# dphoyes/OpenCL-Structure-from-Motion

Hardware: AMD Instinct MI355X
Metric: stereo frame-pairs/sec (1242x375) through pushBack+matchFeatures(2), p_matched bit-exact (higher is better)
Workload: dtype u8

## Files before the change

### opencl-structure-from-motion_amd/csrc/vsm_feat.h

```cpp
#pragma once

#include <stdint.h>

#if defined(__HIPCC__)
#define VF_HD __host__ __device__ __forceinline__
#define VF_HDM __host__ __device__ __forceinline__
#else
#define VF_HD static inline __attribute__((always_inline))
#define VF_HDM inline __attribute__((always_inline))
#endif

typedef short vf_s2 __attribute__((ext_vector_type(2)));

VF_HD uint32_t vf_perm(uint32_t hi, uint32_t lo, uint32_t sel) {
#if defined(__HIP_DEVICE_COMPILE__)
  return __builtin_amdgcn_perm(hi, lo, sel);
#else
  const uint64_t src = ((uint64_t)hi << 32) | lo;
  uint32_t r = 0;
  for (int k = 0; k < 4; k++) {
    const uint32_t s = (sel >> (8 * k)) & 0xffu;
    const uint32_t b = s <= 7u ? (uint32_t)((src >> (8 * s)) & 0xffu) : 0u;
    r |= b << (8 * k);
  }
// ... 279 lines not shown
  const uint32_t t0 = vf_all(dy == 0), t1 = vf_all(dy == 1), t2 = vf_all(dy == 2);
  const uint32_t b3 = vf_all(dyb >= 3), b2 = vf_all(dyb == 2), b1 = vf_all(dyb == 1);
  uint32_t col[5];
#pragma unroll
  for (int c = 0; c < 5; c++) {
    const vf_s2 s2 = vf_pair(R[2][c]), s1 = vf_mm<MAX>(vf_pair(R[1][c]), s2), s0 = vf_mm<MAX>(vf_pair(R[0][c]), s1);
    const vf_s2 p7 = vf_pair(R[7][c]), p8 = vf_mm<MAX>(p7, vf_pair(R[8][c])), p9 = vf_mm<MAX>(p8, vf_pair(R[9][c]));
    const vf_s2 mid = vf_mm<MAX>(vf_mm<MAX>(vf_pair(R[3][c]), vf_pair(R[4][c])), vf_mm<MAX>(vf_pair(R[5][c]), vf_pair(R[6][c])));
    const uint32_t top = vf_bfi(t0, vf_bits(s0), vf_bfi(t1, vf_bits(s1), vf_bfi(t2, vf_bits(s2), neutral)));
    const uint32_t bot = vf_bfi(b3, vf_bits(p9), vf_bfi(b2, vf_bits(p8), vf_bfi(b1, vf_bits(p7), neutral)));
    col[c] = vf_bits(vf_mm<MAX>(vf_mm<MAX>(vf_pair(top), vf_pair(bot)), mid));
  }
  const uint32_t m0 = (vf_all(dx == 0) & 0x0000ffffu) | (vf_all(dx <= 1) & 0xffff0000u), m1 = vf_all(dx <= 2) | 0xffff0000u;
  const uint32_t m3 = vf_all(dxr >= 1) | 0x0000ffffu, m4 = (vf_all(dxr >= 2) & 0x0000ffffu) | (vf_all(dxr >= 3) & 0xffff0000u);
  vf_s2 w = vf_pair(col[2]);
  w = vf_mm<MAX>(w, vf_pair(vf_bfi(m0, col[0], neutral)));
  w = vf_mm<MAX>(w, vf_pair(vf_bfi(m1, col[1], neutral)));
  w = vf_mm<MAX>(w, vf_pair(vf_bfi(m3, col[3], neutral)));
  w = vf_mm<MAX>(w, vf_pair(vf_bfi(m4, col[4], neutral)));
  return MAX ? ((int)w.x > (int)w.y ? (int)w.x : (int)w.y) : ((int)w.x < (int)w.y ? (int)w.x : (int)w.y);
}

template <int STR>
VF_HD void vf_nms_dense_region(const int16_t *f, int li, int lj, int lim_i, int lim_j, int tau, int u0, int v0, int32_t &cmin,
                               int32_t &cmax) {
  static_assert((STR & 1) == 0, "plane rows must stay dword aligned");
  uint32_t R[10][5];
  {
    const uint32_t *base = (const uint32_t *)(f + (lj - 3) * STR + (li - 3));
#pragma unroll
    for (int r = 0; r < 10; r++) {
#pragma unroll
      for (int c = 0; c < 5; c++) R[r][c] = base[r * (STR / 2) + c];
    }
  }
  uint32_t kmin = 0xffffffffu, kmax = 0xffffffffu;
#pragma unroll
  for (int di = 0; di < 4; di++) {
#pragma unroll
    for (int dj = 0; dj < 4; dj++) {
      const int q = 3 + di;
      const uint32_t dw = R[3 + dj][q >> 1];
      const int val = (q & 1) ? ((int)dw >> 16) : (int)(short)(dw & 0xffffu);
      const uint32_t o = (uint32_t)(di * 4 + dj);
      const uint32_t a = ((uint32_t)(val + 32768) << 10) | o, b = ((uint32_t)(32767 - val) << 10) | o;
      kmin = a < kmin ? a : kmin;
      kmax = b < kmax ? b : kmax;
    }
  }
  const int mnv = (int)(kmin >> 10) - 32768, mno = (int)(kmin & 1023u);
  const int mxv = 32767 - (int)(kmax >> 10), mxo = (int)(kmax & 1023u);
  const int dxn = mno >> 2, dyn = mno & 3, dxx = mxo >> 2, dyx = mxo & 3;
  const int cx = lim_i - (li + 3), cy = lim_j - (lj + 3);
  const int wmn = vf_dense_window<false>(R, dxn, dyn, dxn < cx ? dxn : cx, dyn < cy ? dyn : cy);
  const int wmx = vf_dense_window<true>(R, dxx, dyx, dxx < cx ? dxx : cx, dyx < cy ? dyx : cy);
  const bool vmin = (mnv <= -tau) && wmn >= mnv, vmax = (mxv >= tau) && wmx <= mxv;
  cmin = vmin ? (int32_t)(0x80000000u | (uint32_t)(li + dxn + u0) | ((uint32_t)(lj + dyn + v0) << 14)) : 0;
  cmax = vmax ? (int32_t)(0x80000000u | (uint32_t)(li + dxx + u0) | ((uint32_t)(lj + dyx + v0) << 14)) : 0;
}

VF_HD void vf_dense_patch(const uint32_t *s_img, int16_t *s_f, int t, int tx, int ty, int bpl, int h, uint8_t *du_plane,
                          uint8_t *dv_plane, int16_t *dump_f1, int16_t *dump_f2) {
  typedef VfDense G;
  const int pr = t / G::PC, pc = t - pr * G::PC;
  VfWindow<G::ROWS> W;
  vf_load_window<G>(s_img, pc, pr, W);
  const int x0 = tx * G::TW + G::FX + 8 * pc, y0 = ty * G::TH + G::FY + G::ROWS * pr;
  const bool own = pc < G::PC_OWN && pr < G::PR_OWN && x0 >= 0 && x0 < bpl;
  int16_t *f1 = s_f + (G::ROWS * pr) * G::FS + 8 * pc, *f2 = f1 + G::FH * G::FS;
#pragma unroll
  for (int rr = 0; rr < G::ROWS; rr++) {
    const int y = y0 + rr;
    vf_s2 C3[6], C5[6], Cc[6], ctr[4], o1[4], o2[4];
#pragma unroll
    for (int j = 0; j < 6; j++) vf_columns_blob<G::ROWS>(W, rr, j, C3[j], C5[j], Cc[j]);
#pragma unroll
    for (int m = 0; m < 4; m++) ctr[m] = W.pair(rr + 2, m + 1);
    vf_blob_row(C3, C5, Cc, ctr, o1, o2);
    vf_store16(f1 + rr * G::FS, vf_bits(o1[0]), vf_bits(o1[1]), vf_bits(o1[2]), vf_bits(o1[3]));
    vf_store16(f2 + rr * G::FS, vf_bits(o2[0]), vf_bits(o2[1]), vf_bits(o2[2]), vf_bits(o2[3]));
    if (own && y >= 0 && y < h) {
      uint32_t du[2], dv[2];
      vf_s2 S[6], D[6];
#pragma unroll
      for (int j = 0; j < 6; j++) vf_columns_sobel<G::ROWS>(W, rr, j, S[j], D[j]);
      if (y < 3 || y > h - 4) vf_sobel_zero_outside(S, D, y * bpl + x0, 2 * bpl, (h - 2) * bpl);
      vf_sobel_row(S, D, du, dv);
      uint32_t *pu = (uint32_t *)(du_plane + (size_t)y * bpl + x0), *pv = (uint32_t *)(dv_plane + (size_t)y * bpl + x0);
      pu[0] = du[0], pu[1] = du[1];
      pv[0] = dv[0], pv[1] = dv[1];
      if (dump_f1) {
#pragma unroll
        for (int m = 0; m < 4; m++) {
          const int x = x0 + 2 * m;
          dump_f1[(size_t)y * bpl + x] = vf_f1_mask(x, y, bpl, h) ? o1[m].x : (short)0;
          dump_f1[(size_t)y * bpl + x + 1] = vf_f1_mask(x + 1, y, bpl, h) ? o1[m].y : (short)0;
          dump_f2[(size_t)y * bpl + x] = vf_f2_mask(x, y, bpl, h) ? o2[m].x : (short)0;
          dump_f2[(size_t)y * bpl + x + 1] = vf_f2_mask(x + 1, y, bpl, h) ? o2[m].y : (short)0;
        }
      }
    }
  }
}

VF_HD void vf_dense_nms(const int16_t *s_f, int it, int tx, int ty, int mw, int mh, int margin, int tau, int ncu, int ncv,
                        int32_t *cand) {
  typedef VfDense G;
  static_assert(G::CU == 32, "a cell row per half wave");
  const int lcu = it & 31, k = (it >> 5) & 1, lcv = it >> 6;
  const int ci = G::CU * tx + G::CELL_U0 + lcu, cj = G::CV * ty + G::CELL_V0 + lcv;
  const int u0 = tx * G::TW + G::FX, v0 = ty * G::TH + G::FY;
  const int lim_i = mw - 1 - margin - u0, lim_j = mh - 1 - margin - v0;
  int32_t cmin, cmax;
  vf_nms_dense_region<G::FS>(s_f + k * G::FH * G::FS, G::CELL_X0 + (G::N + 1) * lcu, G::CELL_Y0 + (G::N + 1) * lcv, lim_i, lim_j, tau, u0,
                             v0, cmin, cmax);
  if (ci >= 0 && ci < ncu && cj >= 0 && cj < ncv) {
    int32_t *c = cand + (size_t)(ci * ncv + cj) * 4 + 2 * k;
    c[0] = cmin;
    c[1] = cmax;
  }
}

struct VfSparseKeep {
  uint32_t f2[VfSparse::ROWS][4];
};
VF_HD void vf_sparse_patch(const uint32_t *s_img, int16_t *s_f, int t, VfSparseKeep &keep) {
  typedef VfSparse G;
  const int pr = t / G::PC, pc = t - pr * G::PC;
  VfWindow<G::ROWS> W;
  vf_load_window<G>(s_img, pc, pr, W);
  int16_t *f1 = s_f + (G::ROWS * pr) * G::FS + 8 * pc;
#pragma unroll
  for (int rr = 0; rr < G::ROWS; rr++) {
    vf_s2 C3[6], C5[6], Cc[6], ctr[4], o1[4], o2[4];
#pragma unroll
    for (int j = 0; j < 6; j++) vf_columns_blob<G::ROWS>(W, rr, j, C3[j], C5[j], Cc[j]);
#pragma unroll
    for (int m = 0; m < 4; m++) ctr[m] = W.pair(rr + 2, m + 1);
    vf_blob_row(C3, C5, Cc, ctr, o1, o2);
    vf_store16(f1 + rr * G::FS, vf_bits(o1[0]), vf_bits(o1[1]), vf_bits(o1[2]), vf_bits(o1[3]));
#pragma unroll
    for (int m = 0; m < 4; m++) keep.f2[rr][m] = vf_bits(o2[m]);
  }
}
VF_HD void vf_sparse_store_f2(int16_t *s_f, int t, const VfSparseKeep &keep) {
  typedef VfSparse G;
  const int pr = t / G::PC, pc = t - pr * G::PC;
  int16_t *f = s_f + (G::ROWS * pr) * G::FS + 8 * pc;
#pragma unroll
  for (int rr = 0; rr < G::ROWS; rr++) {
    vf_store16(f + rr * G::FS, keep.f2[rr][0], keep.f2[rr][1], keep.f2[rr][2], keep.f2[rr][3]);
  }
}
template <int LANES>
VF_HD void vf_sparse_nms(const int16_t *s_f, int it, int l8, int k, int tx, int ty, int mw, int mh, int margin, int tau, int ncu,
                         int ncv, int32_t *cand) {
  typedef VfSparse G;
  const int lcv = it / G::CU, lcu = it - lcv * G::CU;
  const int ci = G::CU * tx + G::CELL_U0 + lcu, cj = G::CV * ty + G::CELL_V0 + lcv;
  const int u0 = tx * G::TW + G::FX, v0 = ty * G::TH + G::FY;
  const int lim_i = mw - 1 - margin - u0, lim_j = mh - 1 - margin - v0;
  const bool fast = lim_i >= G::FW - 1 && lim_j >= G::FH - 1;
  int32_t cmin, cmax;
  const int li = G::CELL_X0 + (G::N + 1) * lcu, lj = G::CELL_Y0 + (G::N + 1) * lcv;
  if (fast)
    vf_nms_item<G::N, LANES, G::FS, true>(s_f, li, lj, l8, lim_i, lim_j, tau, u0, v0, cmin, cmax);
  else
    vf_nms_item<G::N, LANES, G::FS, false>(s_f, li, lj, l8, lim_i, lim_j, tau, u0, v0, cmin, cmax);
  if (l8 == 0 && ci < ncu && cj < ncv) {
    int32_t *c = cand + (size_t)(ci * ncv + cj) * 4 + 2 * k;
    c[0] = cmin;
    c[1] = cmax;
  }
}
```

### opencl-structure-from-motion_amd/csrc/vsm_image.hip

```cpp

#include <stdlib.h>

#include <algorithm>

#include "vsm_internal.h"
#include "vsm_dev.h"
#include "vsm_feat.h"

#ifdef VSM_FEAT_TIMING
__device__ unsigned int vsm_ft_rec[5][1 << 16][10];
extern "C" int vsm_debug_feat_rec(unsigned int *out, int reset) {
  if (hipMemcpyFromSymbol(out, HIP_SYMBOL(vsm_ft_rec), sizeof(vsm_ft_rec)) != hipSuccess) return -1;
  (void)reset;
  return 0;
}
#define FT_DECL unsigned long long ft_t[10]; int ft_n = 0
#define FT_STAMP ft_t[ft_n++] = __builtin_amdgcn_s_memtime()
#define FT_FLUSH(kern)                                                              \
  do {                                                                              \
    const unsigned wv = ((blockIdx.z * gridDim.y + blockIdx.y) * gridDim.x + blockIdx.x) * (blockDim.x >> 6) + (threadIdx.x >> 6); \
    if ((threadIdx.x & 63) == 0 && wv < (1u << 16)) {                               \
      vsm_ft_rec[kern][wv][0] = (unsigned)ft_t[0] | 1u;                             \
      for (int q = 1; q < ft_n; q++) vsm_ft_rec[kern][wv][q] = (unsigned)(ft_t[q] - ft_t[q - 1]); \
    }                                                                               \
// ... 489 lines not shown
}

template <int N, int TCU, int TCV, int LANES>
__global__ void __launch_bounds__(256)
    k_nms_fixed(const VsmImage *__restrict__ imgs, int first, VsmDims d, const int16_t *__restrict__ f1base,
                const int16_t *__restrict__ f2base, size_t f_stride, int tau, int si, int nbx, int n_img) {
  constexpr int N1 = N + 1, W = 2 * N + 1;
  constexpr int TW = TCU * N1 + 2 * N, TH = TCV * N1 + 2 * N;
  constexpr int STR = (((TW + 1) / 2) | 1) * 2;
  static_assert(TCU * TCV * 2 * LANES == 256, "one item per LANES threads");
  static_assert((N1 & 1) == 0, "tile origins must stay dword aligned");
  __shared__ int16_t s_f[2][TH][STR];
  const int lb = xcd_remap(blockIdx.x, gridDim.x);
  const int zi = lb / nbx, bx = lb - zi * nbx;
  if (zi >= n_img) return;
  const VsmSet &st = imgs[first + zi].set[si];
  const int tiles_u = (st.ncu + TCU - 1) / TCU;
  const int tu = bx % tiles_u, tv = bx / tiles_u;
  const int cu0 = tu * TCU, cv0 = tv * TCV;
  const int u0 = VSM_MARGIN + cu0 * N1, v0 = VSM_MARGIN + cv0 * N1;
  const int16_t *__restrict__ f1 = f1base + (size_t)zi * f_stride;
  const int16_t *__restrict__ f2 = f2base + (size_t)zi * f_stride;
  for (int e = threadIdx.x; e < (TW / 2) * TH; e += 256) {
    const int y = e / (TW / 2), x = 2 * (e - y * (TW / 2));
    const int u = u0 + x, v = v0 + y;
    const bool in = u + 1 < d.mbpl && v < d.mh;
    const uint32_t a = in ? *(const uint32_t *)(f1 + v * d.mbpl + u) : 0u;
    const uint32_t b = in ? *(const uint32_t *)(f2 + v * d.mbpl + u) : 0u;
    *(uint32_t *)&s_f[0][y][x] = a;
    *(uint32_t *)&s_f[1][y][x] = b;
  }
  __syncthreads();
  const int l8 = threadIdx.x % LANES, item = threadIdx.x / LANES;
  const int k = item & 1, cl = item >> 1;
  const int lcu = cl % TCU, lcv = cl / TCU;
  const int ci = cu0 + lcu, cj = cv0 + lcv;
  const bool live = ci < st.ncu && cj < st.ncv;
  const int16_t(*f)[STR] = s_f[k];
  const int li = N + lcu * N1, lj = N + lcv * N1;
  uint32_t kmin = 0xffffffffu, kmax = 0xffffffffu;
  {
    const int16_t *c0 = &f[lj][li];
#pragma unroll
    for (int t = 0; t < (N1 + LANES - 1) / LANES; t++) {
      const int di = l8 + t * LANES;
      if (di < N1) {
#pragma unroll
        for (int dj = 0; dj < N1; dj++) {
          const int val = c0[dj * STR + di];
          const uint32_t o = (uint32_t)(di * N1 + dj);
          kmin = min(kmin, ((uint32_t)(val + 32768) << 10) | o);
          kmax = min(kmax, ((uint32_t)(32767 - val) << 10) | o);
        }
      }
    }
  }
#pragma unroll
  for (int o = LANES / 2; o >= 1; o >>= 1) {
    kmin = min(kmin, (uint32_t)__shfl_xor((int)kmin, o, LANES));
    kmax = min(kmax, (uint32_t)__shfl_xor((int)kmax, o, LANES));
  }
  const int mnv = (int)(kmin >> 10) - 32768, mno = kmin & 1023;
  const int mxv = 32767 - (int)(kmax >> 10), mxo = kmax & 1023;
  const int mni = li + mno / N1, mnj = lj + mno % N1, mxi = li + mxo / N1, mxj = lj + mxo % N1;
  const int lim_i = d.mw - 1 - VSM_MARGIN - u0, lim_j = d.mh - 1 - VSM_MARGIN - v0;
  int wmn = 32767, wmx = -32768;
  if (lim_i >= TW - 1 && lim_j >= TH - 1) {
    typedef short vsm_s2 __attribute__((ext_vector_type(2)));
    constexpr int ND = (W + 1) / 2;
    const int cn = mni - N, cx = mxi - N;
    const bool pn1 = (cn & 1) != 0, px1 = (cx & 1) != 0;
    const uint32_t *pn = (const uint32_t *)&f[mnj - N][cn & ~1], *px = (const uint32_t *)&f[mxj - N][cx & ~1];
    vsm_s2 amn = {32767, 32767}, amx = {-32768, -32768};
#pragma unroll
    for (int t = 0; t < (W + LANES - 1) / LANES; t++) {
      const int r = l8 + t * LANES;
      if (r < W) {
        const uint32_t *rn = pn + r * (STR / 2), *rx = px + r * (STR / 2);
#pragma unroll
        for (int c = 0; c < ND; c++) {
          uint32_t vn = rn[c], vx = rx[c];
          if (c == 0) {
            vn = pn1 ? ((vn & 0xffff0000u) | 0x00007fffu) : vn;
            vx = px1 ? ((vx & 0xffff0000u) | 0x00008000u) : vx;
          }
          if (c == ND - 1) {
            vn = pn1 ? vn : ((vn & 0x0000ffffu) | 0x7fff0000u);
            vx = px1 ? vx : ((vx & 0x0000ffffu) | 0x80000000u);
          }
          amn = __builtin_elementwise_min(amn, __builtin_bit_cast(vsm_s2, vn));
          amx = __builtin_elementwise_max(amx, __builtin_bit_cast(vsm_s2, vx));
        }
      }
    }
    wmn = min((int)amn.x, (int)amn.y);
    wmx = max((int)amx.x, (int)amx.y);
  } else {
    for (int r = l8; r < W; r += LANES) {
      if (mnj - N + r <= lim_j)
        for (int c = 0; c < W && mni - N + c <= lim_i; c++) wmn = min(wmn, (int)f[mnj - N + r][mni - N + c]);
      if (mxj - N + r <= lim_j)
        for (int c = 0; c < W && mxi - N + c <= lim_i; c++) wmx = max(wmx, (int)f[mxj - N + r][mxi - N + c]);
    }
  }
#pragma unroll
  for (int o = LANES / 2; o >= 1; o >>= 1) {
    wmn = min(wmn, __shfl_xor(wmn, o, LANES));
    wmx = max(wmx, __shfl_xor(wmx, o, LANES));
  }
  if (live && l8 == 0) {
    const bool vmin = (mnv <= -tau) && wmn >= mnv, vmax = (mxv >= tau) && wmx <= mxv;
    int32_t *c = st.cand + (size_t)(ci * st.ncv + cj) * 4 + 2 * k;
    c[0] = vmin ? (int32_t)(0x80000000u | (uint32_t)(mni + u0) | ((uint32_t)(mnj + v0) << 14)) : 0;
    c[1] = vmax ? (int32_t)(0x80000000u | (uint32_t)(mxi + u0) | ((uint32_t)(mxj + v0) << 14)) : 0;
  }
}



template <bool DUMP>
__global__ void __launch_bounds__(256)
    k_feat_dense(const VsmImage *__restrict__ imgs, int first, VsmDims d, int tau, int tiles_x, int nbx, int n_img,
                 int16_t *__restrict__ f1base, int16_t *__restrict__ f2base, size_t f_stride) {
  typedef VfDense G;
  __shared__ __attribute__((aligned(16))) uint32_t s_img[G::IH * G::IWD];
  __shared__ __attribute__((aligned(16))) int16_t s_f[2 * G::FH * G::FS];
  const int lb = xcd_remap(blockIdx.x, gridDim.x);
  const int zi = lb / nbx, bx = lb - zi * nbx;
  if (zi >= n_img) return;
  const VsmImage &im = imgs[first + zi];
  const VsmSet &st = im.set[1];
  const int ty = bx / tiles_x, tx = bx - ty * tiles_x;
  const int t = threadIdx.x;
  FT_DECL;
  FT_STAMP;
  vf_fill<G, 256>(s_img, im.imgm, d.mbpl * d.mh, d.mbpl, tx, ty, t);
  FT_STAMP;
  __syncthreads();
  FT_STAMP;
  if (t < G::PC * G::PR)
    vf_dense_patch(s_img, s_f, t, tx, ty, d.mbpl, d.mh, im.du, im.dv, DUMP ? f1base + (size_t)zi * f_stride : nullptr,
                   DUMP ? f2base + (size_t)zi * f_stride : nullptr);
  FT_STAMP;
  __syncthreads();
  FT_STAMP;
  for (int it = t; it < G::CU * G::CV * 2; it += 256) vf_dense_nms(s_f, it, tx, ty, d.mw, d.mh, VSM_MARGIN, tau, st.ncu, st.ncv, st.cand);
  FT_STAMP;
  FT_FLUSH(0);
}

__global__ void __launch_bounds__(256)
    k_feat_sparse(const VsmImage *__restrict__ imgs, int first, VsmDims d, int tau, int tiles_x, int nbx, int n_img) {
  typedef VfSparse G;
  __shared__ __attribute__((aligned(16))) uint32_t s_img[G::IH * G::IWD];
  __shared__ __attribute__((aligned(16))) int16_t s_f[G::FH * G::FS];
  const int lb = xcd_remap(blockIdx.x, gridDim.x);
  const int zi = lb / nbx, bx = lb - zi * nbx;
  if (zi >= n_img) return;
  const VsmImage &im = imgs[first + zi];
  const VsmSet &st = im.set[0];
  const int ty = bx / tiles_x, tx = bx - ty * tiles_x;
  const int t = threadIdx.x;
  FT_DECL;
  FT_STAMP;
  vf_fill<G, 256>(s_img, im.imgm, d.mbpl * d.mh, d.mbpl, tx, ty, t);
  FT_STAMP;
  __syncthreads();
  FT_STAMP;
  VfSparseKeep keep;
  if (t < G::PC * G::PR) vf_sparse_patch(s_img, s_f, t, keep);
  FT_STAMP;
  __syncthreads();
  FT_STAMP;
  static_assert((G::CU * G::CV) % 32 == 0, "whole rounds of 32 items x 8 lanes");
  for (int it = t >> 3; it < G::CU * G::CV; it += 32) vf_sparse_nms<8>(s_f, it, t & 7, 0, tx, ty, d.mw, d.mh, VSM_MARGIN, tau, st.ncu, st.ncv, st.cand);
  FT_STAMP;
  __syncthreads();
  if (t < G::PC * G::PR) vf_sparse_store_f2(s_f, t, keep);
  __syncthreads();
  FT_STAMP;
  for (int it = t >> 3; it < G::CU * G::CV; it += 32) vf_sparse_nms<8>(s_f, it, t & 7, 1, tx, ty, d.mw, d.mh, VSM_MARGIN, tau, st.ncu, st.ncv, st.cand);
  FT_STAMP;
  FT_FLUSH(1);
}

static void vsm_feat_tiles(const VsmDims &d, const VsmSet &dense, int &dx, int &dy) {
  dx = std::max((d.mbpl + 8 + 127) / 128, (dense.ncu + 3 + 31) / 32);
  dy = std::max((d.mh + 4 + 47) / 48, (dense.ncv + 2 + 11) / 12);
}

__global__ void __launch_bounds__(1024) k_scan_cells(const VsmImage *__restrict__ imgs, int first, int set_lo, int nb) {
  __shared__ int s_w[17];
  const VsmSet &st = imgs[first + blockIdx.z].set[blockIdx.y];
  if ((int)blockIdx.y < set_lo) {
    if (threadIdx.x == 0) {
      *st.count = 0;
      *st.count_host = 0;
    }
    return;
  }
  for (int b = threadIdx.x; b < nb; b += 1024) st.bin_cnt[b] = 0;
  const int ncells = st.ncu * st.ncv;
  const int chunk = (ncells + 1023) / 1024;
  const int c0 = min((int)threadIdx.x * chunk, ncells), c1 = min(c0 + chunk, ncells);
  int sum = 0, total, run;
  if (chunk <= 8) {
    int cnt[8];
#pragma unroll
    for (int k = 0; k < 8; k++) {
      cnt[k] = 0;
      if (c0 + k < c1) {
        const int4 v = ldg_i4(st.cand + (size_t)(c0 + k) * 4);
        cnt[k] = (v.x < 0) + (v.y < 0) + (v.z < 0) + (v.w < 0);
      }
    }
#pragma unroll
    for (int k = 0; k < 8; k++) sum += cnt[k];
    run = block_excl_scan_1024(sum, total, s_w);
#pragma unroll
    for (int k = 0; k < 8; k++)
      if (c0 + k < c1) {
        st.cell_off[c0 + k] = run;
        run += cnt[k];
      }
  } else {
    for (int c = c0; c < c1; c++) {
      const int4 v = *(const int4 *)(st.cand + (size_t)c * 4);
      sum += (v.x < 0) + (v.y < 0) + (v.z < 0) + (v.w < 0);
    }
    run = block_excl_scan_1024(sum, total, s_w);
    for (int c = c0; c < c1; c++) {
      const int4 v = *(const int4 *)(st.cand + (size_t)c * 4);
      st.cell_off[c] = run;
      run += (v.x < 0) + (v.y < 0) + (v.z < 0) + (v.w < 0);
    }
  }
  if (threadIdx.x == 0) {
    st.cell_off[ncells] = total;
    *st.count = total;
    *st.count_host = total;
  }
}

__constant__ int8_t c_desc_dv[16] = {-1, +1, -1, +1, -1, +1, -1, +1, -5, +5, -5, +5, -3, +3, -3, +3};
__constant__ int8_t c_desc_du[16] = {-3, -3, -1, -1, +3, +3, +1, +1, -1, -1, +1, +1, -5, -5, +5, +5};

#define EMIT_TW 128
#define EMIT_TH 32
#define EMIT_HALO 5
#define EMIT_LW (EMIT_TW + 2 * EMIT_HALO + 4)
#define EMIT_LH (EMIT_TH + 2 * EMIT_HALO)
__global__ void __launch_bounds__(256) k_emit(const VsmImage *__restrict__ imgs, int first, VsmDims d, int set_lo,
                                              int binsize, int nbx, int n_img) {
  __shared__ uint16_t s_g[EMIT_LH][EMIT_LW + 2];
  const int lb = xcd_remap(blockIdx.x, gridDim.x);
  const int zi = lb / nbx, bx = lb - zi * nbx;
  if (zi >= n_img) return;
  const VsmImage &im = imgs[first + zi];
  const int si = blockIdx.y;
  if (si < set_lo) return;
  const VsmSet &st = im.set[si];
  const int n1 = st.nms_n + 1;
  const int tcu = max(EMIT_TW / n1, 1), tcv = max(EMIT_TH / n1, 1);
  const int tiles_u = (st.ncu + tcu - 1) / tcu, tiles_v = (st.ncv + tcv - 1) / tcv;
  if (bx >= tiles_u * tiles_v) return;
  const int tu = bx % tiles_u, tv = bx / tiles_u;
  const int cu0 = tu * tcu, cv0 = tv * tcv;
  const int ut = st.nms_n + VSM_MARGIN + cu0 * n1 - EMIT_HALO, vt = st.nms_n + VSM_MARGIN + cv0 * n1 - EMIT_HALO;
  const int ua = ut & ~3;
  const bool staged = n1 <= EMIT_TH;
  if (staged) {
    for (int e = threadIdx.x; e < (EMIT_LW / 4 + 1) * EMIT_LH; e += 256) {
      const int y = e / (EMIT_LW / 4 + 1), x = 4 * (e - y * (EMIT_LW / 4 + 1));
      const int u = ua + x, v = vt + y;
      if (x + 3 < EMIT_LW + 2) {
        uint32_t a = 0, b = 0;
        if (u >= 0 && u + 3 < d.mbpl && v >= 0 && v < d.mh) {
          a = ldg_u32(im.du + (size_t)v * d.mbpl + u);
          b = ldg_u32(im.dv + (size_t)v * d.mbpl + u);
        }
        const uint32_t lo = (a & 0xffu) | ((b & 0xffu) << 8) | ((a & 0xff00u) << 8) | ((b & 0xff00u) << 16);
        const uint32_t hi = ((a >> 16) & 0xffu) | (((b >> 16) & 0xffu) << 8) | ((a >> 24) << 16) | ((b >> 24) << 24);
        *(uint2 *)&s_g[y][x] = make_uint2(lo, hi);
      }
    }
    __syncthreads();
  }
  for (int t = threadIdx.x; t < tcu * tcv; t += 256) {
    const int lcv = t % tcv, lcu = t / tcv;
    const int ci = cu0 + lcu, cj = cv0 + lcv;
    if (ci >= st.ncu || cj >= st.ncv) continue;
    const int cell = ci * st.ncv + cj;
    const int4 c4 = ldg_i4(st.cand + (size_t)cell * 4);
    if ((c4.x | c4.y | c4.z | c4.w) >= 0) continue;
    const int cc4[4] = {c4.x, c4.y, c4.z, c4.w};
    int pos = ldg_i32(st.cell_off + cell);
#pragma unroll
    for (int g = 0; g < 4; g++) {
      const int cc = cc4[g];
      if (cc >= 0) continue;
      const int u = cc & 0x3fff, v = (cc >> 14) & 0x3fff;
      uint32_t t16[16];
      if (staged) {
        const uint16_t *c0 = &s_g[v - vt][u - ua];
#pragma unroll
        for (int m = 0; m < 16; m++) {
          constexpr int8_t kdv[16] = {-1, +1, -1, +1, -1, +1, -1, +1, -5, +5, -5, +5, -3, +3, -3, +3};
          constexpr int8_t kdu[16] = {-3, -3, -1, -1, +3, +3, +1, +1, -1, -1, +1, +1, -5, -5, +5, +5};
          t16[m] = c0[kdv[m] * (EMIT_LW + 2) + kdu[m]];
        }
      } else {
#pragma unroll
        for (int m = 0; m < 16; m++) {
          const int a = (v + c_desc_dv[m]) * d.mbpl + u + c_desc_du[m];
          t16[m] = (uint32_t)im.du[a] | ((uint32_t)im.dv[a] << 8);
        }
      }
      vsm_u4 r0, r1, r2;
      r0.x = (uint32_t)(u * d.scale);
      r0.y = (uint32_t)(v * d.scale);
      r0.z = 0u;
      r0.w = (uint32_t)g;
      r1.x = t16[0] | (t16[1] << 16);
      r1.y = t16[2] | (t16[3] << 16);
      r1.z = t16[4] | (t16[5] << 16);
      r1.w = t16[6] | (t16[7] << 16);
      r2.x = t16[8] | (t16[9] << 16);
      r2.y = t16[10] | (t16[11] << 16);
      r2.z = t16[12] | (t16[13] << 16);
      r2.w = t16[14] | (t16[15] << 16);
      VSM_AS1 vsm_u4 *rec = (VSM_AS1 vsm_u4 *)(st.feat + (size_t)pos * 12);
      rec[0] = r0;
      rec[1] = r1;
      rec[2] = r2;
// ... 534 lines not shown
```

Measured before the change: 55100.

## Replace per-cell sparse NMS with hierarchical block-level min/max pruning in shared memory

For interior tiles, the sparse-NMS stage now runs as several cooperative phases. Column min/max reductions feed per-block argmin records, and each cell decides from its 8 neighbour blocks whether it survives. Only ambiguous neighbour regions are queued as jobs for a row scan, and a fallback to the per-item path covers job-buffer overflow. The level structures reuse the image tile's LDS through a union to keep occupancy, at the cost of extra barriers, an atomic job counter and more complex control flow.

```diff
diff --git a/opencl-structure-from-motion_amd/csrc/vsm_feat.h b/opencl-structure-from-motion_amd/csrc/vsm_feat.h
--- a/opencl-structure-from-motion_amd/csrc/vsm_feat.h
+++ b/opencl-structure-from-motion_amd/csrc/vsm_feat.h
@@ -455,24 +455,225 @@
     vf_store16(f + rr * G::FS, keep.f2[rr][0], keep.f2[rr][1], keep.f2[rr][2], keep.f2[rr][3]);
   }
 }
-template <int LANES>
-VF_HD void vf_sparse_nms(const int16_t *s_f, int it, int l8, int k, int tx, int ty, int mw, int mh, int margin, int tau, int ncu,
-                         int ncv, int32_t *cand) {
+VF_HD bool vf_sparse_fast(int tx, int ty, int mw, int mh, int margin) {
+  typedef VfSparse G;
+  return mw - 1 - margin - (tx * G::TW + G::FX) >= G::FW - 1 && mh - 1 - margin - (ty * G::TH + G::FY) >= G::FH - 1;
+}
+template <int LANES, bool fast>
+VF_HD void vf_sparse_item(const int16_t *s_f, int it, int l8, int k, int tx, int ty, int mw, int mh, int margin, int tau, int ncu,
+                          int ncv, int32_t *cand) {
   typedef VfSparse G;
   const int lcv = it / G::CU, lcu = it - lcv * G::CU;
   const int ci = G::CU * tx + G::CELL_U0 + lcu, cj = G::CV * ty + G::CELL_V0 + lcv;
   const int u0 = tx * G::TW + G::FX, v0 = ty * G::TH + G::FY;
   const int lim_i = mw - 1 - margin - u0, lim_j = mh - 1 - margin - v0;
-  const bool fast = lim_i >= G::FW - 1 && lim_j >= G::FH - 1;
   int32_t cmin, cmax;
   const int li = G::CELL_X0 + (G::N + 1) * lcu, lj = G::CELL_Y0 + (G::N + 1) * lcv;
-  if (fast)
-    vf_nms_item<G::N, LANES, G::FS, true>(s_f, li, lj, l8, lim_i, lim_j, tau, u0, v0, cmin, cmax);
-  else
-    vf_nms_item<G::N, LANES, G::FS, false>(s_f, li, lj, l8, lim_i, lim_j, tau, u0, v0, cmin, cmax);
+  vf_nms_item<G::N, LANES, G::FS, fast>(s_f, li, lj, l8, lim_i, lim_j, tau, u0, v0, cmin, cmax);
   if (l8 == 0 && ci < ncu && cj < ncv) {
     int32_t *c = cand + (size_t)(ci * ncv + cj) * 4 + 2 * k;
     c[0] = cmin;
     c[1] = cmax;
   }
 }
+
+typedef uint32_t vf_u2a __attribute__((ext_vector_type(2), may_alias));
+struct alignas(16) VfLevels {
+  typedef VfSparse G;
+  static constexpr int N1 = G::N + 1, BU = G::CU + 2, BV = G::CV + 2, NB = BU * BV, ITEMS = G::CU * G::CV;
+  static constexpr int JOBS = 256;
+  static_assert(G::CELL_X0 - N1 >= 0 && G::CELL_X0 + N1 * (G::CU + 1) <= G::FW, "the ring's columns inside the plane");
+  static_assert(G::CELL_Y0 - G::N == 0 && G::CELL_Y0 + N1 * (G::CV + 1) <= G::FH, "the top ring from row 0, the bottom ring inside the plane");
+  static_assert(G::FS % 4 == 0 && G::FW < 256 && G::FH < 64 && 2 * ITEMS <= 128 && N1 <= 16, "columns in fours; the fields of a block's and a job's word");
+  int16_t col[2][BV][G::FS];
+  uint32_t blk[2][NB];
+  uint32_t jobs[JOBS + 1][2];
+  uint32_t keep[2 * ITEMS];
+  uint32_t full[ITEMS];
+  uint32_t njobs;
+  static VF_HDM int bx0(int bu) { return G::CELL_X0 + N1 * (bu - 1); }
+  static VF_HDM int by0(int bv) { return bv ? G::CELL_Y0 + N1 * (bv - 1) : 0; }
+  static VF_HDM int val16(uint32_t rec, int s) { return (int)(int16_t)(rec & 0xffffu) ^ s; }
+  static VF_HDM int px(uint32_t rec) { return (int)((rec >> 16) & 0xffu); }
+  static VF_HDM int py(uint32_t rec) { return (int)(rec >> 24); }
+};
+VF_HD uint32_t vf_levels_count(uint32_t *p, uint32_t n) {
+#if defined(__HIP_DEVICE_COMPILE__)
+  return atomicAdd(p, n);
+#else
+  const uint32_t v = *p;
+  *p = v + n;
+  return v;
+#endif
+}
+
+template <int NT>
+VF_HD void vf_levels_columns(const int16_t *f, VfLevels &L, int t) {
+  typedef VfLevels V;
+  constexpr int FS = VfSparse::FS, QW = FS / 4;
+  for (int e = t; e < V::BV * QW; e += NT) {
+    const int bv = e / QW, c = e - bv * QW;
+    const int16_t *p = f + V::by0(bv) * FS + 4 * c;
+    vf_u2a r = *(const vf_u2a *)p;
+    vf_s2 mn0 = vf_pair(r.x), mn1 = vf_pair(r.y), mx0 = mn0, mx1 = mn1;
+#pragma unroll
+    for (int i = 1; i < V::N1; i++) {
+      r = *(const vf_u2a *)(p + i * FS);
+      mn0 = __builtin_elementwise_min(mn0, vf_pair(r.x)), mn1 = __builtin_elementwise_min(mn1, vf_pair(r.y));
+      mx0 = __builtin_elementwise_max(mx0, vf_pair(r.x)), mx1 = __builtin_elementwise_max(mx1, vf_pair(r.y));
+    }
+    const vf_u2a mn = {vf_bits(mn0), vf_bits(mn1)}, mx = {vf_bits(mx0), vf_bits(mx1)};
+    *(vf_u2a *)(L.col[0][bv] + 4 * c) = mn;
+    *(vf_u2a *)(L.col[1][bv] + 4 * c) = mx;
+  }
+}
+
+VF_HD void vf_levels_blocks(const int16_t *f, VfLevels &L, int t) {
+  typedef VfLevels V;
+  if (t < V::ITEMS) L.full[t] = 0;
+  if (t == 0) L.njobs = 0;
+  if (t >= 2 * V::NB) return;
+  const int b = t >> 1, k = t & 1, s = -k;
+  const int bv = b / V::BU, bu = b - bv * V::BU;
+  const int x0 = V::bx0(bu), y0 = V::by0(bv);
+  const int16_t *col = L.col[k][bv] + x0;
+  int kx = 0x7fffffff, ky = 0x7fffffff;
+#pragma unroll
+  for (int i = 0; i < V::N1; i++) {
+    const int key = ((int)col[i] ^ s) * 16 + i;
+    kx = key < kx ? key : kx;
+  }
+  const int16_t *line = f + y0 * VfSparse::FS + x0 + (kx & 15);
+#pragma unroll
+  for (int i = 0; i < V::N1; i++) {
+    const int key = ((int)line[i * VfSparse::FS] ^ s) * 16 + i;
+    ky = key < ky ? key : ky;
+  }
+  L.blk[k][b] = ((uint32_t)((ky >> 4) ^ s) & 0xffffu) | ((uint32_t)(x0 + (kx & 15)) << 16) | ((uint32_t)(y0 + (ky & 15)) << 24);
+}
+
+VF_HD void vf_levels_decide(VfLevels &L, int t, int tau) {
+  typedef VfLevels V;
+  if (t >= 2 * V::ITEMS) return;
+  const int it = t >> 1, k = t & 1, s = -k;
+  const int lcv = it / VfSparse::CU, lcu = it - lcv * VfSparse::CU;
+  const uint32_t *blk = L.blk[k] + lcv * V::BU + lcu;
+  const uint32_t own = blk[V::BU + 1];
+  const int v = V::val16(own, s), cx = V::px(own), cy = V::py(own);
+  const int li = V::bx0(lcu + 1), lj = V::by0(lcv + 1), N = VfSparse::N;
+  const int wl = li - cx + N, wr = cx - li, hu = lj - cy + N, hd = cy - lj;
+  const uint32_t xpart[3] = {(uint32_t)(cx - N) | (uint32_t)(wl - 1) << 14, (uint32_t)li | 9u << 14, (uint32_t)(li + V::N1) | (uint32_t)(wr - 1) << 14};
+  const uint32_t ypart[3] = {(uint32_t)(cy - N) << 8 | (uint32_t)(hu - 1) << 18, (uint32_t)lj << 8 | 9u << 18,
+                             (uint32_t)(lj + V::N1) << 8 | (uint32_t)(hd - 1) << 18};
+  const bool some_x[3] = {wl > 0, true, wr > 0}, some_y[3] = {hu > 0, true, hd > 0};
+  bool open = v <= (k ? ~tau : -tau);
+  uint32_t need = 0;
+#pragma unroll
+  for (int n = 0; n < 8; n++) {
+    const int q = n + (n >= 4), du = q % 3, dv = q / 3;
+    const uint32_t r = blk[dv * V::BU + du];
+    const int nx = V::px(r), ny = V::py(r);
+    const bool better = V::val16(r, s) < v;
+    const bool inside = (du == 0 ? nx >= cx - N : du == 2 ? nx <= cx + N : true) && (dv == 0 ? ny >= cy - N : dv == 2 ? ny <= cy + N : true);
+    open = open && !(better && inside);
+    need |= (uint32_t)(better && !inside && some_x[du] && some_y[dv]) << n;
+  }
+  L.keep[t] = open;
+  if (!open || !need) return;
+  const uint32_t base = vf_levels_count(&L.njobs, (uint32_t)__builtin_popcount(need));
+  uint32_t j = base;
+#pragma unroll
+  for (int n = 0; n < 8; n++) {
+    if ((need >> n) & 1u) {
+      const int q = n + (n >= 4);
+      const vf_u2a job = {xpart[q % 3] | ypart[q / 3] | (uint32_t)t << 22, (uint32_t)v};
+      *(vf_u2a *)L.jobs[j < (uint32_t)V::JOBS ? j : (uint32_t)V::JOBS] = job;
+      j++;
+    }
+  }
+  if (j > (uint32_t)V::JOBS) L.full[it] = 1;
+}
+
+template <int NT, int JL>
+VF_HD void vf_levels_scan(const int16_t *f, VfLevels &L, int t) {
+  typedef VfLevels V;
+  const uint32_t nj = L.njobs < (uint32_t)V::JOBS ? L.njobs : (uint32_t)V::JOBS;
+  for (uint32_t j = (uint32_t)(t / JL); j < nj; j += NT / JL) {
+    const vf_u2a jv = *(const vf_u2a *)L.jobs[j];
+    const uint32_t job = jv.x;
+    const int c = (int)(job >> 22), s = -(c & 1), v = (int)jv.y;
+    const int x0 = (int)(job & 0xffu), y0 = (int)((job >> 8) & 0x3fu), w = (int)((job >> 14) & 15u) + 1, h1 = (int)((job >> 18) & 15u);
+    uint32_t mask[V::N1 / 2];
+#pragma unroll
+    for (int i = 0; i < V::N1 / 2; i++) mask[i] = w >= 2 * i + 2 ? 0xffffffffu : (w == 2 * i + 1 ? 0x0000ffffu : 0u);
+    vf_s2 acc = {32767, 32767};
+#pragma unroll
+    for (int rr = 0; rr < (V::N1 + JL - 1) / JL; rr++) {
+      const int r = t % JL + rr * JL;
+      const int16_t *row = f + (y0 + (r < h1 ? r : h1)) * VfSparse::FS + x0;
+#pragma unroll
+      for (int i = 0; i < V::N1 / 2; i++) {
+        uint32_t d;
+        __builtin_memcpy(&d, row + 2 * i, 4);
+        acc = __builtin_elementwise_min(acc, vf_pair(vf_bfi(mask[i], d ^ (uint32_t)s, 0x7fff7fffu)));
+      }
+    }
+    if ((int)acc.x < v || (int)acc.y < v) L.keep[c] = 0;
+  }
+}
+
+template <int NT, int LANES>
+VF_HD void vf_levels_emit(const int16_t *s_f, const VfLevels &L, int t, int k, int tx, int ty, int mw, int mh, int margin, int tau,
+                          int ncu, int ncv, int32_t *cand) {
+  typedef VfLevels V;
+  typedef VfSparse G;
+  const bool over = L.njobs > (uint32_t)V::JOBS;
+  if (t < 2 * V::ITEMS) {
+    const int it = t >> 1, sg = t & 1;
+    const int lcv = it / G::CU, lcu = it - lcv * G::CU;
+    const int ci = G::CU * tx + G::CELL_U0 + lcu, cj = G::CV * ty + G::CELL_V0 + lcv;
+    if (!(over && L.full[it]) && ci < ncu && cj < ncv) {
+      const uint32_t own = L.blk[sg][(lcv + 1) * V::BU + lcu + 1];
+      const uint32_t u = (uint32_t)(V::px(own) + tx * G::TW + G::FX), v = (uint32_t)(V::py(own) + ty * G::TH + G::FY);
+      cand[(size_t)(ci * ncv + cj) * 4 + 2 * k + sg] = L.keep[t] ? (int32_t)(0x80000000u | u | (v << 14)) : 0;
+    }
+  }
+  if (over)
+    for (int it = t / LANES; it < V::ITEMS; it += NT / LANES)
+      if (L.full[it]) vf_sparse_item<LANES, true>(s_f, it, t % LANES, k, tx, ty, mw, mh, margin, tau, ncu, ncv, cand);
+}
+
+#if defined(__HIP_DEVICE_COMPILE__)
+#define VF_PHASE(t, NT, call, barrier) \
+  do {                                 \
+    call;                              \
+    if (barrier) __syncthreads();      \
+  } while (0)
+#else
+#define VF_PHASE(t, NT, call, barrier) \
+  do {                                 \
+    for (t = 0; t < NT; t++) { call; } \
+  } while (0)
+#endif
+template <int NT, int LANES, int JL>
+VF_HD void vf_sparse_levels(const int16_t *s_f, VfLevels &L, int t, int k, int tx, int ty, int mw, int mh, int margin, int tau,
+                            int ncu, int ncv, int32_t *cand) {
+  VF_PHASE(t, NT, vf_levels_columns<NT>(s_f, L, t), true);
+  VF_PHASE(t, NT, vf_levels_blocks(s_f, L, t), true);
+  VF_PHASE(t, NT, vf_levels_decide(L, t, tau), true);
+  VF_PHASE(t, NT, (vf_levels_scan<NT, JL>(s_f, L, t)), true);
+  VF_PHASE(t, NT, (vf_levels_emit<NT, LANES>(s_f, L, t, k, tx, ty, mw, mh, margin, tau, ncu, ncv, cand)), false);
+}
+#undef VF_PHASE
+
+template <int LANES>
+VF_HD void vf_sparse_nms(const int16_t *s_f, int it, int l8, int k, int tx, int ty, int mw, int mh, int margin, int tau, int ncu,
+                         int ncv, int32_t *cand) {
+  if (!vf_sparse_fast(tx, ty, mw, mh, margin)) {
+    vf_sparse_item<LANES, false>(s_f, it, l8, k, tx, ty, mw, mh, margin, tau, ncu, ncv, cand);
+  } else if (it == 0 && l8 == 0) {
+    VfLevels L;
+    for (size_t i = 0; i < sizeof(L); i++) ((uint8_t *)&L)[i] = 0xa5;
+    vf_sparse_levels<256, 1, 1>(s_f, L, 0, k, tx, ty, mw, mh, margin, tau, ncu, ncv, cand);
+  }
+}
diff --git a/opencl-structure-from-motion_amd/csrc/vsm_image.hip b/opencl-structure-from-motion_amd/csrc/vsm_image.hip
--- a/opencl-structure-from-motion_amd/csrc/vsm_image.hip
+++ b/opencl-structure-from-motion_amd/csrc/vsm_image.hip
@@ -665,8 +665,13 @@
 __global__ void __launch_bounds__(256)
     k_feat_sparse(const VsmImage *__restrict__ imgs, int first, VsmDims d, int tau, int tiles_x, int nbx, int n_img) {
   typedef VfSparse G;
-  __shared__ __attribute__((aligned(16))) uint32_t s_img[G::IH * G::IWD];
+  __shared__ __attribute__((aligned(16))) union {
+    uint32_t img[G::IH * G::IWD];
+    VfLevels lv;
+  } s_u;
+  static_assert(sizeof(s_u) == sizeof(s_u.img), "the levels fit the image tile's 12 KB: 34368 bytes of LDS, four workgroups per compute unit");
   __shared__ __attribute__((aligned(16))) int16_t s_f[G::FH * G::FS];
+  uint32_t *const s_img = s_u.img;
   const int lb = xcd_remap(blockIdx.x, gridDim.x);
   const int zi = lb / nbx, bx = lb - zi * nbx;
   if (zi >= n_img) return;
@@ -686,13 +691,20 @@
   __syncthreads();
   FT_STAMP;
   static_assert((G::CU * G::CV) % 32 == 0, "whole rounds of 32 items x 8 lanes");
-  for (int it = t >> 3; it < G::CU * G::CV; it += 32) vf_sparse_nms<8>(s_f, it, t & 7, 0, tx, ty, d.mw, d.mh, VSM_MARGIN, tau, st.ncu, st.ncv, st.cand);
+  const bool fast = vf_sparse_fast(tx, ty, d.mw, d.mh, VSM_MARGIN);
+  if (fast)
+    vf_sparse_levels<256, 8, 4>(s_f, s_u.lv, t, 0, tx, ty, d.mw, d.mh, VSM_MARGIN, tau, st.ncu, st.ncv, st.cand);
+  else
+    for (int it = t >> 3; it < G::CU * G::CV; it += 32) vf_sparse_item<8, false>(s_f, it, t & 7, 0, tx, ty, d.mw, d.mh, VSM_MARGIN, tau, st.ncu, st.ncv, st.cand);
   FT_STAMP;
   __syncthreads();
   if (t < G::PC * G::PR) vf_sparse_store_f2(s_f, t, keep);
   __syncthreads();
   FT_STAMP;
-  for (int it = t >> 3; it < G::CU * G::CV; it += 32) vf_sparse_nms<8>(s_f, it, t & 7, 1, tx, ty, d.mw, d.mh, VSM_MARGIN, tau, st.ncu, st.ncv, st.cand);
+  if (fast)
+    vf_sparse_levels<256, 8, 4>(s_f, s_u.lv, t, 1, tx, ty, d.mw, d.mh, VSM_MARGIN, tau, st.ncu, st.ncv, st.cand);
+  else
+    for (int it = t >> 3; it < G::CU * G::CV; it += 32) vf_sparse_item<8, false>(s_f, it, t & 7, 1, tx, ty, d.mw, d.mh, VSM_MARGIN, tau, st.ncu, st.ncv, st.cand);
   FT_STAMP;
   FT_FLUSH(1);
 }
```

After: 54730. No clear change (-0.7%).
